# rednote-hilab/dots.ocr

Hardware: AMD Instinct MI355X
Metric: pages/sec, dots.ocr 1.7B bf16, A4@200dpi page batch (preprocess + ViT + prefill + 1024-token greedy decode + detokenise) (higher is better)
Workload: dtype bf16; 1 GPU; a4: 8 pages/GPU of 1654x2339 px -> 19824 patches, 5200 prompt tokens/page, max_new_tokens=1024, EOS disabled; pages_per_gpu=8, parallelism=dp1, decode_rows_in_flight=64

## Files before the change

dots_ocr_amd/csrc/engine.hip:

```cpp
#include <hip/hip_runtime.h>
#include <hip/hip_fp16.h>

#include <algorithm>
#include <cmath>
#include <cstdarg>
#include <cstddef>
#include <cstdio>
#include <cstdlib>
#include <cstring>
#include <string>
#include <unordered_map>
#include <vector>

#include "common.h"
#include "decode_layout.h"
#include "dots_ocr_hip.h"
#include "kernels.h"

namespace {

thread_local std::string g_create_error;

struct Tensor {
    bf16_t* p = nullptr;
// ... 38 lines not shown
    else dst[i] = reinterpret_cast<const bf16_t*>(src)[i];
}

__global__ void pad_rows_kernel(const bf16_t* __restrict__ src, bf16_t* __restrict__ dst, int n, int K, int Kpad) {
    const int64_t i = (int64_t)blockIdx.x * 256 + threadIdx.x;
    if (i >= (int64_t)n * Kpad) return;
    const int r = (int)(i / Kpad), c = (int)(i % Kpad);
    dst[i] = c < K ? src[(size_t)r * K + c] : (bf16_t)0;
}

inline int64_t round_up(int64_t a, int64_t b) { return (a + b - 1) / b * b; }

}

hipError_t launch_pack_w13(hipStream_t s, const bf16_t* gate, const bf16_t* up, bf16_t* out, int I, int K) {
    const int64_t n = (int64_t)2 * I * (K / 8);
    hipLaunchKernelGGL(pack_w13_kernel, dim3((unsigned)((n + 255) / 256)), dim3(256), 0, s, gate, up, out, I, K);
    return hipGetLastError();
}
hipError_t launch_convert_to_bf16(hipStream_t s, const void* src, int dtype, bf16_t* dst, int64_t n) {
    hipLaunchKernelGGL(convert_kernel, dim3((unsigned)((n + 255) / 256)), dim3(256), 0, s, src, dtype, dst, n);
    return hipGetLastError();
}

struct DotsEngine {
    DotsConfig cfg{};
    int device = 0;
    hipStream_t stream = nullptr;
    std::string err;
    std::vector<void*> allocs;
    bool finalized = false;

    std::unordered_map<std::string, Tensor> raw;

    bf16_t *patch_w = nullptr, *patch_b = nullptr, *patch_norm = nullptr;
    int patch_k = 0, patch_kpad = 0;
    std::vector<VLayer> vl;
    bf16_t *v_post_norm = nullptr, *m_ln_w = nullptr, *m_ln_b = nullptr, *m0_w = nullptr, *m0_b = nullptr, *m2_w = nullptr, *m2_b = nullptr;
    bf16_t *embed = nullptr, *final_norm = nullptr, *lm_head = nullptr;
    void* lm_head_d = nullptr;
    float *m0_s = nullptr, *m2_s = nullptr, *lm_head_s = nullptr;
    uint8_t *m0_8 = nullptr, *m2_8 = nullptr;
    uint8_t* act_q = nullptr;
    float* act_s = nullptr;
    uint8_t* act_q_v = nullptr;
    float* act_s_v = nullptr;
    hipStream_t s_vit = nullptr, s_dec = nullptr;
    int dec_cus = 128;
    hipEvent_t ev_vis_ready = nullptr, ev_xs = nullptr;
    bf16_t* vis_pref = nullptr;
    int64_t vis_pref_rows = 0;
    bool pref_pending = false;
    bool pref_deferred = false;
    const float* pref_pix = nullptr;
    int64_t pref_patches = 0;
    std::vector<int64_t> pref_grid;
    hipStream_t vs = nullptr;
    hipStream_t s_vit_full = nullptr;
    hipEvent_t ev_tw0 = nullptr, ev_tw_sw = nullptr, ev_dec_end = nullptr;
    int tail_fixed = 0;
    int tail_now = 0;
    int tail_head_blocks = 0;
    uint64_t tw_seq = 0, dec_end_seq = 0, dec_end_at_tw = 0;
    std::vector<LLayer> ll;
    float *v_inv_freq = nullptr, *lm_inv_freq = nullptr;

    int64_t P = 0, Ppad = 0;
    bf16_t *v_xa = nullptr, *v_x = nullptr, *v_xn = nullptr, *v_qkv = nullptr, *v_q = nullptr, *v_k = nullptr, *v_vt = nullptr,
           *v_att = nullptr, *v_act = nullptr, *v_mh = nullptr, *vis = nullptr;
    float* v_pix = nullptr;
    float2* v_cs = nullptr;
    int32_t* v_pos = nullptr;
    Tile64* v_tiles = nullptr;
    QBlock* v_qblocks = nullptr;
    int64_t vis_rows = 0;
    std::vector<int32_t> h_pos;
    std::vector<Tile64> h_tiles;
    std::vector<QBlock> h_qblocks;

    int64_t TP = 0, TPpad = 0;
    bf16_t *p_x = nullptr, *p_xn = nullptr, *p_qkv = nullptr, *p_q = nullptr, *p_k = nullptr, *p_vt = nullptr, *p_att = nullptr, *p_act = nullptr;
    float2* p_cs = nullptr;
    int32_t *p_pos = nullptr, *p_src = nullptr, *p_last = nullptr;
    Tile64* p_tiles = nullptr;
    QBlock* p_qblocks = nullptr;
    std::vector<int32_t> hp_pos, hp_src, hp_last, hp_table;
    std::vector<Tile64> hp_tiles;
    std::vector<QBlock> hp_qblocks;

    int max_pages = 0;
    int n_pool_pages = 0;
    int kv_capped = 0;
    std::vector<int32_t> free_pages;
    std::vector<int32_t> page_refs;
    std::vector<int> fresh_slots;
    int32_t* fk_dev = nullptr;
    std::vector<std::vector<int32_t>> slot_pages;
    bf16_t* pool = nullptr;
    size_t pool_layer_elems = 0;
    bool kv8 = false;
    float* kv_scales = nullptr;
    int32_t *block_table = nullptr, *ctx_len = nullptr, *cur_tokens = nullptr, *out_ids = nullptr, *out_lens = nullptr,
            *finished = nullptr, *eos_ids = nullptr, *am_idx = nullptr;
    float* am_val = nullptr;
    int n_eos = 0;
    float temperature = 0.f, top_p = 1.f;
    uint64_t seed = 0;
    RowParams* d_rowp = nullptr;
    int32_t* d_row_own = nullptr;
    uint32_t* d_row_thr = nullptr;
    int32_t* pen_cnt = nullptr;
    uint32_t* pen_seen = nullptr;
    float* pen_logits = nullptr;
    int row_own[DOTS_MAX_BATCH] = {0};
    int n_own = 0;
    RowRules* d_rules = nullptr;
    float* rule_img = nullptr;
    int32_t *rule_stage = nullptr, *rule_stage_host = nullptr;
    hipEvent_t rule_ev = nullptr;
    int row_rules[DOTS_MAX_BATCH] = {0};
    int n_rules = 0;
    int32_t h_eos[16] = {0};
    int32_t* tok_off = nullptr;
    uint8_t* tok_bytes = nullptr;
    struct Guide { uint16_t* table = nullptr; uint8_t* accepting = nullptr; int n_states = 0, start = 0, rows = 0; };
    std::vector<Guide> guides;
    RowGuide* d_guides = nullptr;
    uint32_t* guide_mask = nullptr;
    int row_guide[DOTS_MAX_BATCH] = {0};
    int n_guided = 0;
    RowNgram* d_ngram = nullptr;
    uint32_t* ngram_mask = nullptr;
    int row_ngram[DOTS_MAX_BATCH] = {0};
    int n_ngram = 0;
    int32_t* d_row_lp = nullptr;
    float *lp_tok = nullptr, *lp_top = nullptr, *lp_ms = nullptr, *lp_pv = nullptr;
    int32_t *lp_ids = nullptr, *lp_pi = nullptr, *lp_pos = nullptr;
    int row_lp[DOTS_MAX_BATCH];
    int n_lp = 0;
    int spec_k = 0, spec_min_n = 0, spec_max_n = 0;
    int32_t *sp_drafts = nullptr, *sp_ndraft = nullptr, *sp_nlive = nullptr, *sp_tokens = nullptr, *sp_ctx = nullptr, *sp_table = nullptr;
    unsigned long long* sp_stats = nullptr;
    int out_cap = 0;
    bf16_t *d_h = nullptr, *d_q = nullptr, *d_att = nullptr, *d_act = nullptr, *d_xn = nullptr;
    float* d_part_h = nullptr;
    float *d_part_o = nullptr, *d_part_ml = nullptr, *d_logits = nullptr;
    int force_part = 0;
    int attn_stream = -1;
    int B = 0;
    int B_sel = 0;
    bool slot_mode = false;
    bool sel_dirty = true;
    int slot_active[DOTS_MAX_BATCH] = {0};
    int slot_limit[DOTS_MAX_BATCH] = {0};
    int slot_prompt[DOTS_MAX_BATCH] = {0};
    int slot_ctx_ub[DOTS_MAX_BATCH] = {0};
    int slot_done[DOTS_MAX_BATCH] = {0};
    int32_t *d_sel = nullptr, *d_sel_new = nullptr, *d_max_len = nullptr, *p_dst = nullptr;
    const int32_t* sel_now = nullptr;
    struct StepGraph { int rows, splits, out_cap, n_eos, part, rowp, lp, rules, guided, ngram, spec; hipGraph_t graph; hipGraphExec_t exec; };
    std::vector<StepGraph> step_graphs;
    std::vector<int> h_prompt_lens;
    int steps_done = 0;

    uint8_t *pp_in = nullptr, *pp_tmp = nullptr, *pp_out = nullptr;
    int32_t* pp_tab = nullptr;
    size_t pp_in_cap = 0, pp_tmp_cap = 0, pp_out_cap = 0, pp_tab_cap = 0;

    bf16_t* dbg_hidden = nullptr;
    size_t dbg_cap = 0;
    int64_t dbg_vit_rows = 0, dbg_lm_rows = 0;

    hipEvent_t ev[8]{};
    std::vector<hipEvent_t> attn_ev;
    DotsStats stats{};
    int attn_pairs = 0;

    int fail(int code, const char* fmt, ...) {
        char buf[1024];
        va_list ap;
        va_start(ap, fmt);
        vsnprintf(buf, sizeof(buf), fmt, ap);
        va_end(ap);
        err = buf;
        return code;
    }
    template <typename T>
    hipError_t alloc(T** p, size_t count) {
        void* q = nullptr;
        hipError_t e = hipMalloc(&q, std::max<size_t>(count * sizeof(T), 256));
        if (e != hipSuccess) return e;
        allocs.push_back(q);
        *p = reinterpret_cast<T*>(q);
        return hipMemsetAsync(q, 0, std::max<size_t>(count * sizeof(T), 256), stream);
    }
    void release(void* p) {
        if (!p) return;
        auto it = std::find(allocs.begin(), allocs.end(), p);
        if (it != allocs.end()) allocs.erase(it);
        hipFree(p);
    }
};

static_assert(sizeof(RowParams) == sizeof(DotsSamplingParams) && offsetof(RowParams, seed) == offsetof(DotsSamplingParams, seed) &&
                  offsetof(RowParams, presence_penalty) == offsetof(DotsSamplingParams, presence_penalty),
              "RowParams (kernels.h) must mirror DotsSamplingParams");

#define CK(expr)                                                                                         \
    do {                                                                                                 \
        hipError_t e_ = (expr);                                                                          \
        if (e_ != hipSuccess) return e->fail(DOTS_E_HIP, "%s failed: %s (%s:%d)", #expr, hipGetErrorString(e_), __FILE__, __LINE__); \
    } while (0)

namespace {

const Tensor* find(DotsEngine* e, const std::string& name) {
    auto it = e->raw.find(name);
    return it == e->raw.end() ? nullptr : &it->second;
}

int need(DotsEngine* e, const std::string& name, std::initializer_list<int64_t> shape, bf16_t** out) {
    const Tensor* t = find(e, name);
    if (!t) return e->fail(DOTS_E_STATE, "missing weight %s", name.c_str());
    if (t->shape != std::vector<int64_t>(shape)) return e->fail(DOTS_E_INVALID, "weight %s has unexpected shape", name.c_str());
    *out = t->p;
    return DOTS_OK;
}

int optional(DotsEngine* e, const std::string& name, std::initializer_list<int64_t> shape, bf16_t** out) {
    const Tensor* t = find(e, name);
    *out = nullptr;
    if (!t) return DOTS_OK;
    if (t->shape != std::vector<int64_t>(shape)) return e->fail(DOTS_E_INVALID, "weight %s has unexpected shape", name.c_str());
    *out = t->p;
    return DOTS_OK;
}

void drop(DotsEngine* e, const std::string& name) {
    auto it = e->raw.find(name);
    if (it == e->raw.end()) return;
    e->release(it->second.p);
    e->raw.erase(it);
}

#define RET(x) do { int r_ = (x); if (r_ != DOTS_OK) return r_; } while (0)

int quantize(DotsEngine* e, bf16_t* W, float** scale, int64_t N, int K, uint8_t** w8 = nullptr) {
    *scale = nullptr;
    if (w8) *w8 = nullptr;
    if (!e->cfg.fp8_weights) return DOTS_OK;
    CK(e->alloc(scale, (size_t)N));
    CK(launch_quant_rows_fp8(e->stream, W, *scale, N, K));
    if (w8) {
        if (!gemm_fp8_supports((int)N, K)) return e->fail(DOTS_E_INVALID, "fp8_weights: a %lld x %d linear does not fit the fp8 GEMM (N %% 256, K %% 64)", (long long)N, K);
        CK(e->alloc(w8, (size_t)N * K));
        CK(launch_bf16q_to_fp8(e->stream, W, *w8, N * K));
    }
    return DOTS_OK;
}

int dense_on(DotsEngine* e, hipStream_t st, uint8_t* aq, float* as, const bf16_t* A, const bf16_t* W, const uint8_t* W8, const float* wscale,
             const bf16_t* bias, const bf16_t* R, void* C, int64_t M, int N, int K, int ldc, int epi) {
    if (!W8) {
        CK(launch_gemm(st, A, W, bias, R, C, M, N, K, K, ldc, epi, wscale));
        return DOTS_OK;
    }
    CK(launch_quant_act_fp8(st, A, aq, as, M, K, K));
    CK(launch_gemm_fp8(st, aq, as, W8, wscale, bias, R, C, M, N, K, ldc, epi));
    return DOTS_OK;
}
int dense(DotsEngine* e, const bf16_t* A, const bf16_t* W, const uint8_t* W8, const float* wscale, const bf16_t* bias, const bf16_t* R, void* C,
          int64_t M, int N, int K, int ldc, int epi) {
    return dense_on(e, e->stream, e->act_q, e->act_s, A, W, W8, wscale, bias, R, C, M, N, K, ldc, epi);
}
int vdense(DotsEngine* e, const bf16_t* A, const bf16_t* W, const uint8_t* W8, const float* wscale, const bf16_t* bias, const bf16_t* R, void* C,
           int64_t M, int N, int K, int ldc, int epi) {
    return dense_on(e, e->vs, e->act_q_v, e->act_s_v, A, W, W8, wscale, bias, R, C, M, N, K, ldc, epi);
}

int qkv_rope_on(DotsEngine* e, hipStream_t st, uint8_t* aq, float* as, const bf16_t* A, const bf16_t* W, const uint8_t* W8, const float* wscale, const bf16_t* bias,
                bf16_t* qkv, const float2* cs, const Tile64* tiles, int n_tiles, bf16_t* q, bf16_t* k, bf16_t* vt, int64_t T, int64_t Tpad, int K, int Hq, int Hkv) {
    const int N = (Hq + 2 * Hkv) * 128;
    if (!W8 && !wscale) {
        const hipError_t r = launch_gemm_qk_rope(st, A, W, bias, qkv, T, N, K, K, N, cs, q, k, Hq, Hkv);
        if (r == hipSuccess) {
            CK(launch_qkv_rope_split(st, qkv, cs, tiles, n_tiles, q, k, vt, T, Tpad, Hq, Hkv, true));
            return DOTS_OK;
        }
        if (r != hipErrorNotSupported) CK(r);
    }
    RET(dense_on(e, st, aq, as, A, W, W8, wscale, bias, nullptr, qkv, T, N, K, N, EPI_NONE));
    CK(launch_qkv_rope_split(st, qkv, cs, tiles, n_tiles, q, k, vt, T, Tpad, Hq, Hkv));
    return DOTS_OK;
}

int decode_copy(DotsEngine* e, const bf16_t* W, void** out, int64_t rows, int K, int rot_rows) {
// ... 113 lines not shown
        CK(hipMemcpyAsync(L.qkv_w + (size_t)Nq * H, kw, (size_t)Nkv * H * 2, hipMemcpyDeviceToDevice, s));
        CK(hipMemcpyAsync(L.qkv_w + (size_t)(Nq + Nkv) * H, vw, (size_t)Nkv * H * 2, hipMemcpyDeviceToDevice, s));
        L.qkv_b = nullptr;
        if (qb && kb && vb) {
            CK(e->alloc(&L.qkv_b, (size_t)(Nq + 2 * Nkv)));
            CK(hipMemcpyAsync(L.qkv_b, qb, (size_t)Nq * 2, hipMemcpyDeviceToDevice, s));
            CK(hipMemcpyAsync(L.qkv_b + Nq, kb, (size_t)Nkv * 2, hipMemcpyDeviceToDevice, s));
            CK(hipMemcpyAsync(L.qkv_b + Nq + Nkv, vb, (size_t)Nkv * 2, hipMemcpyDeviceToDevice, s));
        }
        CK(e->alloc(&L.w13, (size_t)2 * I * H));
        CK(launch_pack_w13(s, gw, uw, L.w13, I, H));
        RET(quantize(e, L.qkv_w, &L.qkv_s, Nq + 2 * Nkv, H, &L.qkv_8));
        RET(quantize(e, L.o_w, &L.o_s, H, Nq, &L.o_8));
        RET(quantize(e, L.w13, &L.w13_s, 2 * I, H, &L.w13_8));
        RET(quantize(e, L.down_w, &L.down_s, H, I, &L.down_8));
        RET(decode_copy(e, L.qkv_w, &L.qkv_wd, Nq + 2 * Nkv, H, Nq + Nkv));
        RET(decode_copy(e, L.o_w, &L.o_wd, H, Nq, 0));
        RET(decode_copy(e, L.w13, &L.w13_wd, 2 * I, H, 0));
        RET(decode_copy(e, L.down_w, &L.down_wd, H, I, 0));
        CK(hipStreamSynchronize(s));
        for (const char* n : {"self_attn.q_proj.weight", "self_attn.k_proj.weight", "self_attn.v_proj.weight",
                              "mlp.gate_proj.weight", "mlp.up_proj.weight"})
            drop(e, p + n);
    }
    {
        std::vector<float> vf(32), lf(64);
        for (int i = 0; i < 32; ++i) vf[i] = 1.0f / powf(10000.0f, (float)(2 * i) / 64.0f);
        for (int i = 0; i < 64; ++i) lf[i] = 1.0f / powf(c.rope_theta, (float)(2 * i) / 128.0f);
        CK(e->alloc(&e->v_inv_freq, 32));
        CK(e->alloc(&e->lm_inv_freq, 64));
        CK(hipMemcpyAsync(e->v_inv_freq, vf.data(), 32 * 4, hipMemcpyHostToDevice, s));
        CK(hipMemcpyAsync(e->lm_inv_freq, lf.data(), 64 * 4, hipMemcpyHostToDevice, s));
        CK(hipStreamSynchronize(s));
    }
    e->finalized = true;
    return DOTS_OK;
}

int alloc_workspaces(DotsEngine* e) {
    const DotsConfig& c = e->cfg;
    const int E = c.v_embed_dim, H = c.hidden_size, Nq = c.num_heads * 128, Nkv = c.num_kv_heads * 128;
    const int Mg = E * c.v_merge * c.v_merge;
    e->P = c.max_patches;
    e->Ppad = e->P + 64 * 256;
    const int kpad = (int)round_up(c.v_channels * c.v_patch * c.v_patch, 64);
    if (c.fp8_weights) {
        const size_t v_max = (size_t)e->P * std::max(E, c.v_intermediate);
        const size_t p_max = (size_t)c.max_prefill_tokens * std::max(H, std::max(Nq, c.intermediate_size));
        CK(e->alloc(&e->act_q, p_max));
        CK(e->alloc(&e->act_s, (size_t)c.max_prefill_tokens));
        CK(e->alloc(&e->act_q_v, v_max));
        CK(e->alloc(&e->act_s_v, (size_t)e->P));
    }
    CK(e->alloc(&e->v_xa, (size_t)e->P * kpad));
    CK(e->alloc(&e->v_x, (size_t)e->P * E));
    CK(e->alloc(&e->v_xn, (size_t)e->P * E));
    CK(e->alloc(&e->v_qkv, (size_t)e->P * 3 * E));
    CK(e->alloc(&e->v_q, (size_t)e->P * E));
    CK(e->alloc(&e->v_k, (size_t)(e->P + 64) * E));
    CK(e->alloc(&e->v_vt, (size_t)e->Ppad * E));
    CK(e->alloc(&e->v_att, (size_t)e->P * E));
    CK(e->alloc(&e->v_act, (size_t)e->P * c.v_intermediate));
    CK(e->alloc(&e->v_mh, (size_t)(e->P / 4 + 1) * Mg));
    CK(e->alloc(&e->vis, (size_t)(e->P / 4 + 1) * H));
    CK(e->alloc(&e->vis_pref, (size_t)(e->P / 4 + 1) * H));
    CK(e->alloc(&e->v_cs, (size_t)e->P * 64));
    CK(e->alloc(&e->v_pos, (size_t)e->P * 2));
    CK(e->alloc(&e->v_tiles, (size_t)(e->P / 64 + 256)));
    CK(e->alloc(&e->v_qblocks, (size_t)(e->P / 128 + 256) * c.v_heads));

    e->TP = c.max_prefill_tokens;
    e->TPpad = e->TP + 64 * c.max_batch;
    CK(e->alloc(&e->p_x, (size_t)e->TP * H));
    CK(e->alloc(&e->p_xn, (size_t)e->TP * H));
    CK(e->alloc(&e->p_qkv, (size_t)e->TP * (Nq + 2 * Nkv)));
    CK(e->alloc(&e->p_q, (size_t)e->TP * Nq));
    CK(e->alloc(&e->p_k, (size_t)(e->TP + 64) * Nkv));
    CK(e->alloc(&e->p_vt, (size_t)e->TPpad * Nkv));
    CK(e->alloc(&e->p_att, (size_t)e->TP * Nq));
    CK(e->alloc(&e->p_act, (size_t)e->TP * c.intermediate_size));
    CK(e->alloc(&e->p_cs, (size_t)e->TP * 64));
    CK(e->alloc(&e->p_pos, (size_t)e->TP));
    CK(e->alloc(&e->p_src, (size_t)e->TP));
    CK(e->alloc(&e->p_last, (size_t)DOTS_MAX_BATCH));
    CK(e->alloc(&e->p_tiles, (size_t)(e->TP / 64 + c.max_batch + 1)));
    CK(e->alloc(&e->p_qblocks, (size_t)(e->TP / 128 + c.max_batch + 1) * c.num_heads));

    e->max_pages = (c.max_seq_len + 63) / 64;
    const int64_t pool_tokens = c.kv_pool_tokens > 0 ? c.kv_pool_tokens : (int64_t)c.max_batch * e->max_pages * 64;
    e->n_pool_pages = (int)((pool_tokens + 63) / 64);
    e->kv8 = c.kv_cache_dtype == 1;
    e->pool_layer_elems = (size_t)(e->n_pool_pages + 1) * c.num_kv_heads * 2 * 8192 / (e->kv8 ? 2 : 1);
    CK(e->alloc(&e->pool, e->pool_layer_elems * c.num_layers));
    const std::vector<float> kv_ones((size_t)c.num_layers * c.num_kv_heads * 2, 1.0f);
    CK(e->alloc(&e->kv_scales, kv_ones.size()));
    CK(hipMemcpyAsync(e->kv_scales, kv_ones.data(), kv_ones.size() * 4, hipMemcpyHostToDevice, e->stream));
    const int mb = (c.max_batch + 15) / 16 * 16;
    CK(e->alloc(&e->block_table, (size_t)mb * e->max_pages));
    CK(e->alloc(&e->ctx_len, (size_t)mb));
    CK(e->alloc(&e->cur_tokens, (size_t)mb));
    CK(e->alloc(&e->out_ids, (size_t)mb * c.max_seq_len));
    CK(e->alloc(&e->out_lens, (size_t)mb));
    CK(e->alloc(&e->finished, (size_t)mb));
    CK(e->alloc(&e->eos_ids, (size_t)16));
    CK(e->alloc(&e->d_sel, (size_t)DOTS_MAX_BATCH));
    CK(e->alloc(&e->d_sel_new, (size_t)DOTS_MAX_BATCH));
    CK(e->alloc(&e->d_max_len, (size_t)DOTS_MAX_BATCH));
    CK(e->alloc(&e->p_dst, (size_t)DOTS_MAX_BATCH));
    CK(e->alloc(&e->fk_dev, (size_t)3 * DOTS_MAX_BATCH));
    CK(e->alloc(&e->am_idx, (size_t)mb * 64));
    CK(e->alloc(&e->am_val, (size_t)mb * 64));
    CK(e->alloc(&e->d_h, (size_t)mb * H));
    CK(e->alloc(&e->d_q, (size_t)mb * Nq));
    CK(e->alloc(&e->d_att, (size_t)mb * Nq));
    CK(e->alloc(&e->d_act, (size_t)mb * c.intermediate_size));
    CK(e->alloc(&e->d_xn, (size_t)DOTS_MAX_BATCH * H));
    CK(e->alloc(&e->d_part_h, (size_t)DEC_KSPLIT_PARTS * DOTS_MAX_BATCH * H));
    CK(e->alloc(&e->d_logits, (size_t)mb * c.vocab_size));
    CK(e->alloc(&e->d_part_o, (size_t)mb * c.num_heads * 64 * 128));
    CK(e->alloc(&e->d_part_ml, (size_t)mb * c.num_heads * 64 * 2));
    if (const char* fm = getenv("DOTS_OCR_DECODE_PLAN")) {
        const int plan = atoi(fm);
        if (plan < 0 || plan > 5 || (plan & 6) == 6) {
            fprintf(stderr, "dots.ocr: DOTS_OCR_DECODE_PLAN=%s ignored: must be 0 / 1 (partition plan on every step), + 2 (streaming attention) or + 4 (per-split attention)\n", fm);
        } else {
            e->force_part = plan & 1;
            e->attn_stream = (plan & 2) ? 1 : (plan & 4) ? 0 : -1;
        }
    }
    if (const char* v = getenv("DOTS_OCR_TOWER_TAIL_LAYERS")) e->tail_fixed = std::max(-1, std::min(atoi(v), c.v_layers));
    e->hp_table.assign((size_t)mb * e->max_pages, e->n_pool_pages);
    e->slot_pages.assign(mb, {});
    e->free_pages.resize(e->n_pool_pages);
    e->page_refs.assign(e->n_pool_pages, 0);
    for (int p = 0; p < e->n_pool_pages; ++p) e->free_pages[p] = e->n_pool_pages - 1 - p;
    CK(hipMemcpyAsync(e->block_table, e->hp_table.data(), e->hp_table.size() * 4, hipMemcpyHostToDevice, e->stream));
    for (auto& ev : e->ev) CK(hipEventCreate(&ev));
    CK(hipStreamSynchronize(e->stream));
    return DOTS_OK;
}

const float* layer_kv_scales(const DotsEngine* e, int layer) {
    return e->kv8 ? e->kv_scales + (size_t)layer * e->cfg.num_kv_heads * 2 : nullptr;
}

hipError_t upload_table_row(DotsEngine* e, int slot) {
    return hipMemcpyAsync(e->block_table + (size_t)slot * e->max_pages, e->hp_table.data() + (size_t)slot * e->max_pages, (size_t)e->max_pages * 4,
                          hipMemcpyHostToDevice, e->stream);
}
void release_pages(DotsEngine* e, int slot) {
    auto& mine = e->slot_pages[slot];
    for (auto it = mine.rbegin(); it != mine.rend(); ++it)
        if (--e->page_refs[*it] == 0) e->free_pages.push_back(*it);
    mine.clear();
    std::fill(e->hp_table.begin() + (size_t)slot * e->max_pages, e->hp_table.begin() + (size_t)(slot + 1) * e->max_pages, e->n_pool_pages);
}
bool reserve_pages(DotsEngine* e, int slot, int tokens) {
    const int need = (tokens + 63) / 64;
    if (need > (int)e->free_pages.size() || need > e->max_pages) return false;
    auto& mine = e->slot_pages[slot];
    for (int p = 0; p < need; ++p) {
        mine.push_back(e->free_pages.back());
        e->free_pages.pop_back();
        e->page_refs[mine.back()] = 1;
        e->hp_table[(size_t)slot * e->max_pages + p] = mine.back();
    }
    return true;
}

// ... 460 lines not shown
    if (head_ms <= 0.f) return e->tail_now;
    const float t_block = head_ms / (float)e->tail_head_blocks;
    const int tail = d_ms <= 0.f ? L / 2 : (int)floorf((float)L - d_ms / t_block);
    return std::max(0, std::min(tail, L / 2));
}

int chain_streams(DotsEngine* e, hipStream_t from, hipStream_t to) {
    if (from == to) return DOTS_OK;
    CK(hipEventRecord(e->ev_xs, from));
    CK(hipStreamWaitEvent(to, e->ev_xs, 0));
    return DOTS_OK;
}

int pick_decode_stream(DotsEngine* e, hipStream_t* cur) {
    hipStream_t want = e->stream;
    if (e->s_vit && e->pref_pending && !e->pref_deferred && hipEventQuery(e->ev_vis_ready) == hipErrorNotReady) {
        (void)hipGetLastError();
        want = e->s_dec;
    }
    if (want != *cur) {
        RET(chain_streams(e, *cur, want));
        *cur = want;
    }
    return DOTS_OK;
}

int stage_pixels(DotsEngine* e, hipStream_t st, const float* pixel_values, int on_device, int64_t total_patches, const float** pix) {
    *pix = pixel_values;
    if (!on_device) {
        if (total_patches > e->P) return e->fail(DOTS_E_CAPACITY, "total_patches exceeds max_patches");
        if (!e->v_pix) CK(e->alloc(&e->v_pix, (size_t)e->P * e->patch_k));
        CK(hipMemcpyAsync(e->v_pix, pixel_values, (size_t)total_patches * e->patch_k * 4, hipMemcpyHostToDevice, st));
        *pix = e->v_pix;
    }
    return DOTS_OK;
}

int launch_prefetched_tower(DotsEngine* e) {
    e->pref_deferred = false;
    e->tail_now = pick_tower_tail(e);
    e->dec_end_at_tw = e->dec_end_seq;
    ++e->tw_seq;
    RET(chain_streams(e, e->stream, e->s_vit));
    e->vs = e->s_vit;
    int r = vit_forward(e, e->pref_pix, e->pref_patches, e->pref_grid.data(), (int)(e->pref_grid.size() / 3), nullptr, e->vis_pref, &e->vis_pref_rows);
    e->vs = e->stream;
    if (e->s_vit_full) {
        const int rc = chain_streams(e, e->s_vit_full, e->s_vit);
        if (r == DOTS_OK) r = rc;
    }
    CK(hipEventRecord(e->ev_vis_ready, e->s_vit));
    if (r != DOTS_OK) e->pref_pending = false;
    return r;
}

int prefill(DotsEngine* e, const int32_t* ids, const int32_t* lens, int B, const int32_t* slots = nullptr, const int32_t* max_new = nullptr) {
    const DotsConfig& c = e->cfg;
    hipStream_t s = e->stream;
    const int H = c.hidden_size, Hq = c.num_heads, Hkv = c.num_kv_heads, Nq = Hq * 128, Nkv = Hkv * 128, NQKV = Nq + 2 * Nkv;
    if (B < 1 || B > c.max_batch) return e->fail(DOTS_E_CAPACITY, "batch %d exceeds max_batch %d", B, c.max_batch);
    int64_t T = 0;
    std::vector<int> L(B), S(B);
    int rows = B;
    for (int b = 0; b < B; ++b) {
        if (lens[b] < 1 || lens[b] >= c.max_seq_len) return e->fail(DOTS_E_CAPACITY, "prompt %d length %d not in [1, max_seq_len)", b, lens[b]);
        L[b] = lens[b];
        T += lens[b];
        S[b] = slots ? slots[b] : b;
        if (slots) {
            if (S[b] < 0 || S[b] >= c.max_batch) return e->fail(DOTS_E_INVALID, "slot %d out of range [0, %d)", S[b], c.max_batch);
            if (e->spec_k && S[b] >= c.max_batch / (e->spec_k + 1))
                return e->fail(DOTS_E_CAPACITY, "slot %d is not usable while speculating: with %d drafts a slot takes %d rows of a step, so only slots [0, max_batch / (k + 1)) = [0, %d) are",
                               S[b], e->spec_k, e->spec_k + 1, c.max_batch / (e->spec_k + 1));
            if (e->slot_mode && e->slot_active[S[b]]) return e->fail(DOTS_E_STATE, "slot %d is occupied", S[b]);
            for (int a = 0; a < b; ++a)
                if (S[a] == S[b]) return e->fail(DOTS_E_INVALID, "slot %d listed twice", S[b]);
            if (max_new[b] < 1 || lens[b] + max_new[b] > c.max_seq_len)
                return e->fail(DOTS_E_CAPACITY, "slot %d: prompt (%d) + max_new_tokens (%d) exceeds max_seq_len %d", S[b], lens[b], max_new[b], c.max_seq_len);
            rows = std::max(rows, S[b] + 1);
        }
    }
    if (T > e->TP) return e->fail(DOTS_E_CAPACITY, "packed prompt tokens %lld > max_prefill_tokens %lld", (long long)T, (long long)e->TP);
    e->fresh_slots.clear();
    e->hp_pos.resize(T); e->hp_src.resize(T); e->hp_last.assign(DOTS_MAX_BATCH, 0);
    int64_t t = 0, vis_used = 0;
    for (int b = 0; b < B; ++b) {
        for (int i = 0; i < L[b]; ++i, ++t) {
            e->hp_pos[t] = i;
            const int id = ids[t];
            if (id == c.image_token_id) e->hp_src[t] = -(int32_t)(++vis_used);
            else if (id < 0 || id >= c.vocab_size) return e->fail(DOTS_E_INVALID, "token id %d out of range", id);
            else e->hp_src[t] = id;
        }
        e->hp_last[b] = (int32_t)(t - 1);
    }
    if (vis_used != (vis_used ? e->vis_rows : 0))
        return e->fail(DOTS_E_STATE, "prompt has %lld image tokens but the vision tower produced %lld rows", (long long)vis_used, (long long)e->vis_rows);
    int64_t Tpad = 0;
    build_worklists(L, Hq, e->hp_tiles, e->hp_qblocks, &Tpad, S.data());
    CK(hipMemcpyAsync(e->p_pos, e->hp_pos.data(), T * 4, hipMemcpyHostToDevice, s));
    CK(hipMemcpyAsync(e->p_src, e->hp_src.data(), T * 4, hipMemcpyHostToDevice, s));
    CK(hipMemcpyAsync(e->p_last, e->hp_last.data(), DOTS_MAX_BATCH * 4, hipMemcpyHostToDevice, s));
    CK(hipMemcpyAsync(e->p_tiles, e->hp_tiles.data(), e->hp_tiles.size() * sizeof(Tile64), hipMemcpyHostToDevice, s));
    CK(hipMemcpyAsync(e->p_qblocks, e->hp_qblocks.data(), e->hp_qblocks.size() * sizeof(QBlock), hipMemcpyHostToDevice, s));
    if (!slots || !e->slot_mode)
        for (int b = 0; b < (int)e->slot_pages.size(); ++b) release_pages(e, b);
    const bool whole_table = !slots || !e->slot_mode;
    {
        int need = 0;
        for (int b = 0; b < B; ++b) need += ((slots ? admit_tokens(e, L[b], max_new[b]) : std::min(L[b] + e->out_cap, c.max_seq_len)) + 63) / 64;
        if (need > (int)e->free_pages.size()) {
            const int have = (int)e->free_pages.size();
            if (whole_table) CK(hipMemcpyAsync(e->block_table, e->hp_table.data(), e->hp_table.size() * 4, hipMemcpyHostToDevice, s));
            return e->fail(DOTS_E_CAPACITY, "KV pool exhausted: these sequences need %d pages of 64 tokens, %d of %d are free", need, have, e->n_pool_pages);
        }
        for (int b = 0; b < B; ++b) reserve_pages(e, S[b], slots ? admit_tokens(e, L[b], max_new[b]) : std::min(L[b] + e->out_cap, c.max_seq_len));
        if (whole_table) CK(hipMemcpyAsync(e->block_table, e->hp_table.data(), e->hp_table.size() * 4, hipMemcpyHostToDevice, s));
        else for (int b = 0; b < B; ++b) CK(upload_table_row(e, S[b]));
    }
    struct PageGuard {
        DotsEngine* e; const std::vector<int>& S; bool slots, armed = true;
        ~PageGuard() {
            if (!armed || !slots) return;
            for (int sl : S) { release_pages(e, sl); (void)upload_table_row(e, sl); }
        }
    } page_guard{e, S, slots != nullptr};
    if (!slots) {
        e->slot_mode = false;
        std::fill(e->slot_active, e->slot_active + DOTS_MAX_BATCH, 0);
        CK(hipMemcpyAsync(e->ctx_len, lens, B * 4, hipMemcpyHostToDevice, s));
        CK(hipMemsetAsync(e->out_lens, 0, c.max_batch * 4, s));
        CK(hipMemsetAsync(e->finished, 0, c.max_batch * 4, s));
    } else {
        if (!e->slot_mode) {
            std::fill(e->slot_active, e->slot_active + DOTS_MAX_BATCH, 0);
            CK(hipMemsetAsync(e->ctx_len, 0, c.max_batch * 4, s));
            e->slot_mode = true;
        }
        int32_t sel_new[DOTS_MAX_BATCH] = {0};
        for (int b = 0; b < B; ++b) {
            sel_new[S[b]] = 1;
            CK(hipMemcpyAsync(e->ctx_len + S[b], lens + b, 4, hipMemcpyHostToDevice, s));
            CK(hipMemcpyAsync(e->d_max_len + S[b], max_new + b, 4, hipMemcpyHostToDevice, s));
            CK(hipMemsetAsync(e->out_lens + S[b], 0, 4, s));
            CK(hipMemsetAsync(e->finished + S[b], 0, 4, s));
            if (e->sp_ndraft) {
                CK(hipMemsetAsync(e->sp_ndraft + S[b], 0, 4, s));
                CK(hipMemsetAsync(e->sp_stats + (size_t)S[b] * 3, 0, 3 * sizeof(unsigned long long), s));
            }
        }
        CK(hipMemcpyAsync(e->d_sel_new, sel_new, DOTS_MAX_BATCH * 4, hipMemcpyHostToDevice, s));
        CK(hipMemcpyAsync(e->p_dst, S.data(), B * 4, hipMemcpyHostToDevice, s));
    }

    for (int b = 0; b < B; ++b) RET(clear_lp_row(e, S[b]));
    CK(hipEventRecord(e->ev[2], s));
    CK(launch_embed_gather(s, e->p_src, e->embed, e->vis, e->p_x, T, H));
    CK(launch_rope_table(s, e->p_pos, e->lm_inv_freq, e->p_cs, T, 0));
    const float scale = 1.0f / sqrtf(128.0f);
    const int n_tiles = (int)e->hp_tiles.size();
    for (int i = 0; i < c.num_layers; ++i) {
        const LLayer& Lw = e->ll[i];
        bf16_t* pool_l = e->pool + e->pool_layer_elems * i;
        CK(launch_rmsnorm(s, e->p_x, Lw.ln1, e->p_xn, T, H, c.rms_norm_eps));
        RET(qkv_rope_on(e, s, e->act_q, e->act_s, e->p_xn, Lw.qkv_w, Lw.qkv_8, Lw.qkv_s, Lw.qkv_b, e->p_qkv, e->p_cs, e->p_tiles, n_tiles, e->p_q, e->p_k, e->p_vt, T, Tpad, H, Hq, Hkv));
        CK(launch_kv_to_pages(s, e->p_k, e->p_qkv, e->p_tiles, n_tiles, e->block_table, e->max_pages, pool_l, T, Hq, Hkv, layer_kv_scales(e, i)));
        CK(launch_flash_attn(s, e->p_q, e->p_k, e->p_vt, e->p_att, e->p_qblocks, (int)e->hp_qblocks.size(), T, Tpad, Hq, Hkv, 1, scale));
        RET(dense(e, e->p_att, Lw.o_w, Lw.o_8, Lw.o_s, nullptr, e->p_x, e->p_x, T, H, Nq, H, EPI_RESIDUAL));
        CK(launch_rmsnorm(s, e->p_x, Lw.ln2, e->p_xn, T, H, c.rms_norm_eps));
        RET(dense(e, e->p_xn, Lw.w13, Lw.w13_8, Lw.w13_s, nullptr, nullptr, e->p_act, T, 2 * c.intermediate_size, H, c.intermediate_size, EPI_SWIGLU));
        RET(dense(e, e->p_act, Lw.down_w, Lw.down_8, Lw.down_s, nullptr, e->p_x, e->p_x, T, H, c.intermediate_size, H, EPI_RESIDUAL));
        const size_t voff = (size_t)c.v_layers * e->dbg_vit_rows * c.v_embed_dim;
        if (e->dbg_hidden && voff + (size_t)(i + 1) * T * H <= e->dbg_cap) {
            CK(hipMemcpyAsync(e->dbg_hidden + voff + (size_t)i * T * H, e->p_x, (size_t)T * H * 2, hipMemcpyDeviceToDevice, s));
            e->dbg_lm_rows = T;
        }
    }
    if (e->pen_cnt) CK(launch_pen_prompt(s, e->p_src, e->p_last, slots ? e->p_dst : nullptr, B, c.image_token_id, c.vocab_size, e->pen_cnt, e->pen_seen));
    if (e->n_guided > 0) CK(launch_guide_reset_rows(s, e->d_guides, slots ? e->p_dst : nullptr, B));
    CK(launch_gather_rows(s, e->p_x, e->p_last, slots ? e->p_dst : nullptr, e->d_h, B, H));
    CK(launch_dec_lmhead(s, e->d_h, e->final_norm, e->lm_head_d, e->lm_head_s, e->d_logits, rows, H, c.vocab_size, c.rms_norm_eps));
    e->B_sel = rows;
    e->sel_now = e->d_sel_new;
    RET(select_tokens(e, 0));
    CK(hipEventRecord(e->ev[3], s));
    if (slots) {
        for (int b = 0; b < B; ++b) {
            e->slot_active[S[b]] = 1;
            e->slot_limit[S[b]] = L[b] + max_new[b];
            e->slot_prompt[S[b]] = L[b];
            e->slot_ctx_ub[S[b]] = L[b];
            e->slot_done[S[b]] = 0;
        }
        e->sel_dirty = true;
        e->B = 0;
        e->fresh_slots = S;
    } else {
        e->B = B;
        e->h_prompt_lens = L;
    }
    page_guard.armed = false;
    if (e->pref_deferred) RET(launch_prefetched_tower(e));
    e->steps_done = 0;
    e->vis_rows = 0;
    e->stats.prefill_tokens = T;
    double pf = 0;
    const double lin = (double)c.num_layers * ((double)H * NQKV + (double)Nq * H + 3.0 * H * c.intermediate_size);
    for (int b = 0; b < B; ++b) pf += 2.0 * lin * L[b] + (double)c.num_layers * 2.0 * L[b] * (double)L[b] * Nq + 2.0 * (double)c.vocab_size * H;
    e->stats.prefill_flops = pf;
    return DOTS_OK;
}

int decode_step_launches(DotsEngine* e, int n_splits, int part = 0) {
    const DotsConfig& c = e->cfg;
    hipStream_t s = e->stream;
    const int H = c.hidden_size, Hq = c.num_heads, Hkv = c.num_kv_heads, Nq = Hq * 128, I = c.intermediate_size;
    const int rows = e->B, spec_k = e->slot_mode ? e->spec_k : 0;
    const int B = rows * (spec_k + 1);
    const float scale = 1.0f / sqrtf(128.0f);
    const int32_t *tokens = e->cur_tokens, *ctx_len = e->ctx_len, *block_table = e->block_table;
    const SpecState sp = spec_state(e);
    if (spec_k) {
        CK(launch_spec_expand(s, sp, step_state(e, 1, e->d_sel), e->block_table, e->max_pages, rows, e->n_pool_pages));
        tokens = e->sp_tokens; ctx_len = e->sp_ctx; block_table = e->sp_table;
    }
    CK(launch_dec_embed(s, tokens, e->embed, e->d_h, B, H));
    if (e->force_part) part = 1;
    static const bool same_layer = getenv("DOTS_OCR_DEBUG_SAME_LAYER") != nullptr;
    bool pend = false;
    const float* pend_scale = nullptr;
    for (int i = 0; i < c.num_layers; ++i) {
        const LLayer& L = e->ll[same_layer ? 0 : i];
        bf16_t* pool_l = e->pool + e->pool_layer_elems * i;
        CK(launch_dec_qkv(s, e->d_h, L.ln1, L.qkv_wd, L.qkv_s, L.qkv_b, e->lm_inv_freq, ctx_len, block_table, e->max_pages, pool_l, e->d_q, B, H, Hq,
                          Hkv, c.rms_norm_eps, part ? e->dec_cus : 0, e->d_xn, pend ? e->d_part_h : nullptr, pend_scale, layer_kv_scales(e, i)));
        CK(launch_decode_attn(s, e->d_q, pool_l, ctx_len, block_table, e->max_pages, e->d_part_o, e->d_part_ml, B, Hq, Hkv, n_splits, scale, part ? e->dec_cus : 0, e->attn_stream,
                              layer_kv_scales(e, i)));
        CK(launch_decode_attn_combine(s, e->d_part_o, e->d_part_ml, ctx_len, e->d_att, B, Hq, Hkv, n_splits));
        bool pend_o = false;
        CK(launch_dec_proj(s, e->d_att, L.o_wd, L.o_s, e->d_h, B, H, Nq, part ? e->dec_cus : 0, e->d_part_h, &pend_o));
        CK(launch_dec_gateup(s, e->d_h, L.ln2, L.w13_wd, L.w13_s, e->d_act, B, H, I, c.rms_norm_eps, part ? e->dec_cus : 0, e->d_xn, pend_o ? e->d_part_h : nullptr, L.o_s));
        CK(launch_dec_proj(s, e->d_act, L.down_wd, L.down_s, e->d_h, B, H, I, part ? e->dec_cus : 0, e->d_part_h, &pend));
        pend_scale = L.down_s;
    }
    CK(launch_dec_lmhead(s, e->d_h, e->final_norm, e->lm_head_d, e->lm_head_s, e->d_logits, B, H, c.vocab_size, c.rms_norm_eps, part ? e->dec_cus : 0, e->d_xn,
                         pend ? e->d_part_h : nullptr, pend_scale));
    if (spec_k) CK(launch_spec_argmax(s, sp, e->d_logits, c.vocab_size, c.vocab_size, rows, e->am_val, e->am_idx));
    e->B_sel = rows;
    e->sel_now = e->d_sel;
    RET(select_tokens(e, 1));
    if (spec_k) {
        const StepState st = step_state(e, 1, e->d_sel);
        CK(launch_spec_accept(s, sp, st, rows, e->am_val, e->am_idx));
        if (e->spec_max_n > 0)
            CK(launch_ngram_draft(s, st.out_ids, st.out_lens, st.out_stride, st.finished, st.sel, sp.own, sp.lp, sp.engine_greedy, rows, spec_k, e->spec_min_n,
                                  e->spec_max_n, e->sp_drafts, DOTS_MAX_SPEC_DRAFTS, e->sp_ndraft));
    }
    return DOTS_OK;
}

int splits_for_ctx(int max_ctx) { return decode_attn_splits(max_ctx); }

int step_graph(DotsEngine* e, int rows, int n_splits, int out_cap, hipGraphExec_t* exec, int part = 0) {
// ... 1749 lines not shown
```

dots_ocr_amd/csrc/kernels.h:

```cpp
#pragma once
#include <hip/hip_runtime.h>
#include <stdint.h>

typedef uint16_t bf16_t;

#define DOTS_MAX_BATCH 64

enum { EPI_NONE = 0, EPI_RESIDUAL = 1, EPI_SWIGLU = 2, EPI_GELU = 3, EPI_F32 = 4, EPI_QKROPE = 5  };

hipError_t launch_gemm(hipStream_t s, const bf16_t* A, const bf16_t* W, const bf16_t* bias, const bf16_t* R,
                       void* C, int64_t M, int N, int K, int lda, int ldc, int epi, const float* colscale = nullptr);
int gemm_get_plan();
void gemm_set_plan(int plan);

hipError_t launch_rmsnorm(hipStream_t s, const bf16_t* x, const bf16_t* w, bf16_t* y, int64_t rows, int dim, float eps);
hipError_t launch_layernorm(hipStream_t s, const bf16_t* x, const bf16_t* w, const bf16_t* b, bf16_t* y,
                            int64_t rows, int dim, float eps);
hipError_t launch_patch_prep(hipStream_t s, const float* x, bf16_t* y, int64_t rows, int in_dim, int out_dim);
hipError_t launch_rope_table(hipStream_t s, const int32_t* pos, const float* inv_freq, float2* cs, int64_t T, int two_d);
struct Tile64 { int32_t tok0, n, pad0, seq, page, _pad; };
hipError_t launch_qkv_rope_split(hipStream_t s, const bf16_t* qkv, const float2* cs, const Tile64* tiles, int n_tiles,
                                 bf16_t* q, bf16_t* k, bf16_t* vt, int64_t T, int64_t Tpad, int Hq, int Hkv, bool v_only = false);
struct QkRope { const float2* cs; bf16_t* q; bf16_t* k; long long T; int Hq; int n_rope_heads; };
hipError_t launch_gemm_qk_rope(hipStream_t s, const bf16_t* A, const bf16_t* W, const bf16_t* bias, bf16_t* qkv, int64_t M, int N, int K, int lda, int ldc,
                               const float2* cs, bf16_t* q, bf16_t* k, int Hq, int Hkv);
hipError_t launch_embed_gather(hipStream_t s, const int32_t* src, const bf16_t* embed, const bf16_t* vision, bf16_t* x,
                               int64_t T, int dim);
hipError_t launch_gather_rows(hipStream_t s, const bf16_t* x, const int32_t* rows, const int32_t* dst, bf16_t* y, int n, int dim);

struct QBlock { int32_t q0, n, tok0, pad0, head, _pad; };
int flash_rows_per_block();
struct XcdPlan { int32_t base[8], cnt[8]; };
XcdPlan make_xcd_plan(const QBlock* blocks_host, int n_blocks);
hipError_t launch_flash_attn(hipStream_t s, const bf16_t* q, const bf16_t* k, const bf16_t* vt, bf16_t* out,
                             const QBlock* blocks, int n_blocks, int64_t T, int64_t Tpad, int Hq, int Hkv,
                             int causal, float scale, const XcdPlan* plan = nullptr);

hipError_t launch_kv_to_pages(hipStream_t s, const bf16_t* k, const bf16_t* qkv, const Tile64* tiles, int n_tiles,
                              const int32_t* block_table, int max_pages, void* pool_layer, int64_t T, int Hq, int Hkv,
                              const float* kv_scales = nullptr);
hipError_t launch_kv_fork_pages(hipStream_t s, void* pool, size_t layer_bytes, size_t page_bytes, int layers, int src_page, const int32_t* dst_pages,
                                int n);
hipError_t launch_dec_embed(hipStream_t s, const int32_t* tokens, const bf16_t* embed, bf16_t* h, int B, int dim);
hipError_t launch_dec_qkv(hipStream_t s, const bf16_t* h, const bf16_t* ln_w, const void* Wd, const float* wscale, const bf16_t* bias,
                          const float* inv_freq, const int32_t* ctx_len, const int32_t* block_table, int max_pages,
                          void* pool_layer, bf16_t* q_out, int B, int H, int Hq, int Hkv, float eps, int part_cus = 0, bf16_t* xn = nullptr,
                          const float* pend = nullptr, const float* pend_scale = nullptr, const float* kv_scales = nullptr);
hipError_t launch_dec_proj(hipStream_t s, const bf16_t* X, const void* Wd, const float* wscale, bf16_t* h, int B, int N, int K, int part_cus = 0,
                           float* part = nullptr, bool* pending = nullptr);
hipError_t launch_dec_gateup(hipStream_t s, const bf16_t* h, const bf16_t* ln_w, const void* W13d, const float* wscale, bf16_t* act,
                             int B, int H, int I, float eps, int part_cus = 0, bf16_t* xn = nullptr, const float* pend = nullptr, const float* pend_scale = nullptr);
hipError_t launch_dec_lmhead(hipStream_t s, const bf16_t* h, const bf16_t* ln_w, const void* Wd, const float* wscale, float* logits,
                             int B, int H, int V, float eps, int part_cus = 0, bf16_t* xn = nullptr, const float* pend = nullptr, const float* pend_scale = nullptr);
bool dec_stream64_supports(int B, int H);
hipError_t launch_dec_norm_ximg(hipStream_t s, const bf16_t* h, const bf16_t* ln_w, bf16_t* xn, int B, int H, float eps, const float* part = nullptr, const float* pscale = nullptr);
hipError_t launch_dec_gateup64(hipStream_t s, const bf16_t* h, const bf16_t* ln_w, const void* W13d, const float* wscale, bf16_t* act, bf16_t* xn,
                               int B, int H, int I, float eps, int cus, const float* pend = nullptr, const float* pend_scale = nullptr);
hipError_t launch_dec_lmhead64(hipStream_t s, const bf16_t* h, const bf16_t* ln_w, const void* Wd, const float* wscale, float* logits, bf16_t* xn,
                               int B, int H, int V, float eps, int cus, const float* pend = nullptr, const float* pend_scale = nullptr);
constexpr int DEC_KSPLIT_PARTS = 4;
bool dec_proj_ksplit_supports(int B, int N, int K);
hipError_t launch_dec_proj_ksplit(hipStream_t s, const bf16_t* X, const void* Wd, bool fp8, float* part, int B, int N, int K, int cus);
int decode_attn_waves();
int decode_attn_splits(int max_seq_len);
hipError_t launch_decode_attn(hipStream_t s, const bf16_t* q, const void* pool_layer, const int32_t* ctx_len,
                              const int32_t* block_table, int max_pages, float* part_o, float* part_ml,
                              int B, int Hq, int Hkv, int n_splits, float scale, int part_cus = 0, int stream_mode = -1,
                              const float* kv_scales = nullptr);
int decode_attn_stream_wgs(int B, int Hkv, int n_splits, int max_pages, int part_cus, int stream_mode = -1, bool kv8 = false);
hipError_t launch_decode_attn_combine(hipStream_t s, const float* part_o, const float* part_ml, const int32_t* ctx_len, bf16_t* out,
                                      int B, int Hq, int Hkv, int n_splits);
struct StepState {
    int32_t *cur_tokens, *ctx_len, *out_ids, *out_lens, *finished;
    const int32_t *eos_ids, *sel, *max_len;
    int n_eos, out_stride, cap, advance_ctx;
};
hipError_t launch_argmax_step(hipStream_t s, const float* logits, int V, int ld, int B, float* pval, int32_t* pidx, const StepState& st);
hipError_t launch_sample_step(hipStream_t s, const float* logits, int V, int ld, int B, float temperature, float top_p, uint64_t seed,
                              const StepState& st, const int32_t* own = nullptr);
struct RowParams { float temperature, top_p; int32_t top_k; float repetition_penalty, frequency_penalty, presence_penalty; uint64_t seed; };
#ifndef DOTS_MAX_STOP_IDS
#define DOTS_MAX_STOP_IDS 16
#endif
enum { RULE_ON = 1, RULE_IMG = 2, RULE_IGNORE_EOS = 4 };
struct RowRules { int32_t flags, min_tokens, n_stop, stop[DOTS_MAX_STOP_IDS]; };
constexpr uint16_t GUIDE_DEAD = 0xFFFF;
struct RowGuide { const uint16_t* table; const uint8_t* accepting; int32_t n_states, start, state, _pad; };
struct GuideSel { RowGuide* rows; uint32_t* mask; const int32_t* tok_off; const uint8_t* tok_bytes; int32_t words, V; };
inline int guide_mask_words(int V) { return ((V + 63) / 64) * 2; }
#ifndef DOTS_MAX_NGRAM_SIZE
#define DOTS_MAX_NGRAM_SIZE 64
#endif
#ifndef DOTS_MAX_NGRAM_WHITELIST
#define DOTS_MAX_NGRAM_WHITELIST 16
#endif
struct RowNgram { int32_t n, window, n_white, white[DOTS_MAX_NGRAM_WHITELIST]; };
struct NgramSel { const RowNgram* rows; uint32_t* mask; int32_t words, V; };
inline int ngram_mask_words(int V) { return (V + 31) / 32; }
constexpr int NGRAM_MAX_V = 64 * 1024 * 8;
struct RowSel {
    const RowParams* params;
    const int32_t* own;
    int32_t* cnt;
    const uint32_t* seen;
    float* pen;
    uint32_t* thr;
    int legacy_greedy;
    const RowRules* rules;
    const float* rule_img;
    GuideSel guide;
    NgramSel ngram;
};
hipError_t launch_select_rows(hipStream_t s, const float* logits, int V, int ld, int B, const RowSel& rs, float* pval, int32_t* pidx, const StepState& st);
hipError_t launch_pen_prompt(hipStream_t s, const int32_t* src, const int32_t* last, const int32_t* dst, int B, int image_token, int V,
                             int32_t* cnt, uint32_t* seen);
hipError_t launch_pen_history(hipStream_t s, const int32_t* hist, const int32_t* hist_lens, int stride, const int32_t* n_prompt, int B, int V,
                              int32_t* cnt, uint32_t* seen, int32_t* out_lens);
hipError_t launch_set_row_params(hipStream_t s, RowParams* table, int32_t* own, int row, const RowParams& p, int flag);
hipError_t launch_set_row_rules(hipStream_t s, RowRules* table, float* img, int row, int V, const RowRules& r, const int32_t* allowed, int n_allowed,
// ... 68 lines not shown
```

Baseline: 6.150 pages/s.

## Compute only last-token rows in final prefill layer after attention

In the final decoder layer of prefill, attention runs only over the query blocks holding each sequence's last token. Those rows and their residuals are gathered into small per-batch buffers, and o-proj, MLP and norm run on B rows instead of all T prompt tokens. The KV for the last layer is still written in full, so decode is unaffected. An env var or hidden-state capture restores the full computation. This saves about one layer's o-proj and MLP over roughly 41k tokens, at the cost of extra bookkeeping.

```diff
diff --git a/dots_ocr_amd/csrc/engine.hip b/dots_ocr_amd/csrc/engine.hip
--- a/dots_ocr_amd/csrc/engine.hip
+++ b/dots_ocr_amd/csrc/engine.hip
@@ -144,6 +144,7 @@
     bf16_t *p_x = nullptr, *p_xn = nullptr, *p_qkv = nullptr, *p_q = nullptr, *p_k = nullptr, *p_vt = nullptr, *p_att = nullptr, *p_act = nullptr;
     float2* p_cs = nullptr;
     int32_t *p_pos = nullptr, *p_src = nullptr, *p_last = nullptr;
+    bf16_t *pl_x = nullptr, *pl_xn = nullptr, *pl_att = nullptr, *pl_act = nullptr;
     Tile64* p_tiles = nullptr;
     QBlock* p_qblocks = nullptr;
     std::vector<int32_t> hp_pos, hp_src, hp_last, hp_table;
@@ -274,6 +275,12 @@
         if (e_ != hipSuccess) return e->fail(DOTS_E_HIP, "%s failed: %s (%s:%d)", #expr, hipGetErrorString(e_), __FILE__, __LINE__); \
     } while (0)
 
+bool prefill_full_last_layer(bool hidden_capture) {
+    if (hidden_capture) return true;
+    const char* v = getenv("DOTS_OCR_PREFILL_FULL_LAST");
+    return v && atoi(v) != 0;
+}
+
 namespace {
 
 const Tensor* find(DotsEngine* e, const std::string& name) {
@@ -553,9 +560,13 @@
     CK(e->alloc(&e->p_cs, (size_t)e->TP * 64));
     CK(e->alloc(&e->p_pos, (size_t)e->TP));
     CK(e->alloc(&e->p_src, (size_t)e->TP));
-    CK(e->alloc(&e->p_last, (size_t)DOTS_MAX_BATCH));
+    CK(e->alloc(&e->p_last, (size_t)2 * DOTS_MAX_BATCH));
+    CK(e->alloc(&e->pl_x, (size_t)c.max_batch * H));
+    CK(e->alloc(&e->pl_xn, (size_t)c.max_batch * H));
+    CK(e->alloc(&e->pl_att, (size_t)c.max_batch * Nq));
+    CK(e->alloc(&e->pl_act, (size_t)c.max_batch * c.intermediate_size));
     CK(e->alloc(&e->p_tiles, (size_t)(e->TP / 64 + c.max_batch + 1)));
-    CK(e->alloc(&e->p_qblocks, (size_t)(e->TP / 128 + c.max_batch + 1) * c.num_heads));
+    CK(e->alloc(&e->p_qblocks, (size_t)(e->TP / 128 + 2 * c.max_batch + 1) * c.num_heads));
 
     e->max_pages = (c.max_seq_len + 63) / 64;
     const int64_t pool_tokens = c.kv_pool_tokens > 0 ? c.kv_pool_tokens : (int64_t)c.max_batch * e->max_pages * 64;
@@ -1182,7 +1193,8 @@
     }
     if (T > e->TP) return e->fail(DOTS_E_CAPACITY, "packed prompt tokens %lld > max_prefill_tokens %lld", (long long)T, (long long)e->TP);
     e->fresh_slots.clear();
-    e->hp_pos.resize(T); e->hp_src.resize(T); e->hp_last.assign(DOTS_MAX_BATCH, 0);
+    e->hp_pos.resize(T); e->hp_src.resize(T); e->hp_last.assign(2 * DOTS_MAX_BATCH, 0);
+    for (int b = 0; b < DOTS_MAX_BATCH; ++b) e->hp_last[DOTS_MAX_BATCH + b] = b;
     int64_t t = 0, vis_used = 0;
     for (int b = 0; b < B; ++b) {
         for (int i = 0; i < L[b]; ++i, ++t) {
@@ -1198,9 +1210,17 @@
         return e->fail(DOTS_E_STATE, "prompt has %lld image tokens but the vision tower produced %lld rows", (long long)vis_used, (long long)e->vis_rows);
     int64_t Tpad = 0;
     build_worklists(L, Hq, e->hp_tiles, e->hp_qblocks, &Tpad, S.data());
+    const bool full_last = prefill_full_last_layer(e->dbg_hidden != nullptr);
+    const int n_qb = (int)e->hp_qblocks.size();
+    if (!full_last)
+        for (int i = 0; i < n_qb; ++i) {
+            const QBlock qb = e->hp_qblocks[i];
+            if (qb.q0 + flash_rows_per_block() >= qb.n) e->hp_qblocks.push_back(qb);
+        }
+    const int n_qb_last = (int)e->hp_qblocks.size() - n_qb;
     CK(hipMemcpyAsync(e->p_pos, e->hp_pos.data(), T * 4, hipMemcpyHostToDevice, s));
     CK(hipMemcpyAsync(e->p_src, e->hp_src.data(), T * 4, hipMemcpyHostToDevice, s));
-    CK(hipMemcpyAsync(e->p_last, e->hp_last.data(), DOTS_MAX_BATCH * 4, hipMemcpyHostToDevice, s));
+    CK(hipMemcpyAsync(e->p_last, e->hp_last.data(), 2 * DOTS_MAX_BATCH * 4, hipMemcpyHostToDevice, s));
     CK(hipMemcpyAsync(e->p_tiles, e->hp_tiles.data(), e->hp_tiles.size() * sizeof(Tile64), hipMemcpyHostToDevice, s));
     CK(hipMemcpyAsync(e->p_qblocks, e->hp_qblocks.data(), e->hp_qblocks.size() * sizeof(QBlock), hipMemcpyHostToDevice, s));
     if (!slots || !e->slot_mode)
@@ -1265,7 +1285,17 @@
         CK(launch_rmsnorm(s, e->p_x, Lw.ln1, e->p_xn, T, H, c.rms_norm_eps));
         RET(qkv_rope_on(e, s, e->act_q, e->act_s, e->p_xn, Lw.qkv_w, Lw.qkv_8, Lw.qkv_s, Lw.qkv_b, e->p_qkv, e->p_cs, e->p_tiles, n_tiles, e->p_q, e->p_k, e->p_vt, T, Tpad, H, Hq, Hkv));
         CK(launch_kv_to_pages(s, e->p_k, e->p_qkv, e->p_tiles, n_tiles, e->block_table, e->max_pages, pool_l, T, Hq, Hkv, layer_kv_scales(e, i)));
-        CK(launch_flash_attn(s, e->p_q, e->p_k, e->p_vt, e->p_att, e->p_qblocks, (int)e->hp_qblocks.size(), T, Tpad, Hq, Hkv, 1, scale));
+        if (i == c.num_layers - 1 && !full_last) {
+            CK(launch_flash_attn(s, e->p_q, e->p_k, e->p_vt, e->p_att, e->p_qblocks + n_qb, n_qb_last, T, Tpad, Hq, Hkv, 1, scale));
+            CK(launch_gather_rows(s, e->p_att, e->p_last, nullptr, e->pl_att, B, Nq));
+            CK(launch_gather_rows(s, e->p_x, e->p_last, nullptr, e->pl_x, B, H));
+            RET(dense(e, e->pl_att, Lw.o_w, Lw.o_8, Lw.o_s, nullptr, e->pl_x, e->pl_x, B, H, Nq, H, EPI_RESIDUAL));
+            CK(launch_rmsnorm(s, e->pl_x, Lw.ln2, e->pl_xn, B, H, c.rms_norm_eps));
+            RET(dense(e, e->pl_xn, Lw.w13, Lw.w13_8, Lw.w13_s, nullptr, nullptr, e->pl_act, B, 2 * c.intermediate_size, H, c.intermediate_size, EPI_SWIGLU));
+            RET(dense(e, e->pl_act, Lw.down_w, Lw.down_8, Lw.down_s, nullptr, e->pl_x, e->pl_x, B, H, c.intermediate_size, H, EPI_RESIDUAL));
+            break;
+        }
+        CK(launch_flash_attn(s, e->p_q, e->p_k, e->p_vt, e->p_att, e->p_qblocks, n_qb, T, Tpad, Hq, Hkv, 1, scale));
         RET(dense(e, e->p_att, Lw.o_w, Lw.o_8, Lw.o_s, nullptr, e->p_x, e->p_x, T, H, Nq, H, EPI_RESIDUAL));
         CK(launch_rmsnorm(s, e->p_x, Lw.ln2, e->p_xn, T, H, c.rms_norm_eps));
         RET(dense(e, e->p_xn, Lw.w13, Lw.w13_8, Lw.w13_s, nullptr, nullptr, e->p_act, T, 2 * c.intermediate_size, H, c.intermediate_size, EPI_SWIGLU));
@@ -1278,7 +1308,8 @@
     }
     if (e->pen_cnt) CK(launch_pen_prompt(s, e->p_src, e->p_last, slots ? e->p_dst : nullptr, B, c.image_token_id, c.vocab_size, e->pen_cnt, e->pen_seen));
     if (e->n_guided > 0) CK(launch_guide_reset_rows(s, e->d_guides, slots ? e->p_dst : nullptr, B));
-    CK(launch_gather_rows(s, e->p_x, e->p_last, slots ? e->p_dst : nullptr, e->d_h, B, H));
+    if (full_last) CK(launch_gather_rows(s, e->p_x, e->p_last, slots ? e->p_dst : nullptr, e->d_h, B, H));
+    else CK(launch_gather_rows(s, e->pl_x, e->p_last + DOTS_MAX_BATCH, slots ? e->p_dst : nullptr, e->d_h, B, H));
     CK(launch_dec_lmhead(s, e->d_h, e->final_norm, e->lm_head_d, e->lm_head_s, e->d_logits, rows, H, c.vocab_size, c.rms_norm_eps));
     e->B_sel = rows;
     e->sel_now = e->d_sel_new;
diff --git a/dots_ocr_amd/csrc/kernels.h b/dots_ocr_amd/csrc/kernels.h
--- a/dots_ocr_amd/csrc/kernels.h
+++ b/dots_ocr_amd/csrc/kernels.h
@@ -35,6 +35,8 @@
 hipError_t launch_flash_attn(hipStream_t s, const bf16_t* q, const bf16_t* k, const bf16_t* vt, bf16_t* out,
                              const QBlock* blocks, int n_blocks, int64_t T, int64_t Tpad, int Hq, int Hkv,
                              int causal, float scale, const XcdPlan* plan = nullptr);
+
+bool prefill_full_last_layer(bool hidden_capture);
 
 hipError_t launch_kv_to_pages(hipStream_t s, const bf16_t* k, const bf16_t* qkv, const Tile64* tiles, int n_tiles,
                               const int32_t* block_table, int max_pages, void* pool_layer, int64_t T, int Hq, int Hkv,
```

After: 6.162 pages/s, median of 6. Within noise of the previous version (+0.2%).
